# PhilipPragerUrbina/DOGERAY

Measured on AMD Instinct MI355X. Metric: Mrays/sec + ms/frame, 1M-tri .rts at 1920x1080, higher is better.
Workload: dtype f32

## Files before the change

### dogeray_amd/csrc/context.cpp

```cpp
#include <climits>
#include <exception>

#include "context.hpp"
#include "linearise.hpp"

using namespace dr;

namespace {

constexpr int ANY = INT_MIN;
struct Option { const char* name; int dr_context::*member; int lo, hi; unsigned only; bool reorders; };
const Option OPTIONS[] = {
    {"kernel", &dr_context::kernel, DR_KERNEL_TILE, DR_KERNEL_PERSISTENT, 0, false},
    {"occupancy", &dr_context::occupancy, 4, 6, 0, false},
    {"schedule", &dr_context::schedule, 0, 2, 0, false},
    {"heavy_factor", &dr_context::heavy_factor, -1, 1000, 0, true},
    {"coop_steps", &dr_context::coop_steps, 0, INT_MAX, 0, false},
    {"coop_lanes", &dr_context::coop_lanes, 1, 64, 0, false},
    {"split_parts", &dr_context::split_parts, 1, 8, 1u << 1 | 1u << 2 | 1u << 4 | 1u << 8, false},
    {"split_waves", &dr_context::split_waves, 1, 1000, 0, true},
    {"split_steps", &dr_context::split_steps, 16, 4080, 0, true},
    {"short_one_queue", &dr_context::short_one_queue, ANY, 0, 0, true},
    {"coop_rounds", &dr_context::coop_rounds, 1, 16, 0, false},
    {"reserve_cus", &dr_context::reserve_cus, 0, 64, 0, false},
    {"wave_log", &dr_context::wave_log_on, 0, 1, 0, false},
    {"coop_tiles_per_wave", &dr_context::coop_tiles_per_wave, 0, INT_MAX, 0, false},
    {"pipe_streams", &dr_context::pipe_streams, 2, dr_context::PIPE_STREAMS, 0, false},
    {"pipe_lean", &dr_context::pipe_lean, ANY, 0, 0, false},
    {"pipe_group", &dr_context::pipe_group, 1, dr_context::PIPE_GROUP_MAX, 0, false},
    {"xcd_regions", &dr_context::xcd_regions, ANY, 0, 0, true},
    {"batch_frames", &dr_context::batch_frames, 1, 256, 0, false},
    {"feedback", &dr_context::feedback, ANY, 0, 0, true},
    {"order_follows_camera", &dr_context::order_follows_camera, ANY, 0, 0, false},
    {"feedback_every", &dr_context::feedback_every, 1, INT_MAX, 0, false},
    {"wide_tree", &dr_context::wide_tree, 0, 2, 0, false},
    {"denoise_tiles", &dr_context::denoise_tiles, 0, 1, 0, false},
    {"moments", &dr_context::moments_opt, 0, 1, 0, false},
    {"denoise_variance", &dr_context::denoise_variance, 0, 1, 0, false},
    {"camera_cert", &dr_context::camera_cert, 0, 1, 0, false},
    {"cert_factor", &dr_context::cert_factor, 1, 10000, 0, false},
    {"cert_levels",  &dr_context::cert_levels, 0, 1, 0, false},
    {"camera_entry",  &dr_context::camera_entry, 0, 1, 0, false},
    {"sky_tiles",  &dr_context::sky_tiles, 0, 1, 0, false},
    {"trace_kernel",  &dr_context::trace_kernel, 0, 2, 0, false},
};

const Option* find_option(const std::string& name) {
  for (const Option& o : OPTIONS) if (name == o.name) return &o;
  return nullptr;
}

int set_option(dr_context* c, const std::string& name, int v) {
  const Option* o = find_option(name);
  if (!o) { set_error("unknown option '" + name + "'"); return DR_ERR_INVALID; }
  if (o->lo == ANY) v = v != 0;
  else if (v < o->lo || v > o->hi || (o->only && !(o->only >> v & 1u))) { set_error("value not supported for option '" + name + "'"); return DR_ERR_INVALID; }
  if (name == "split_steps") v &= ~15;
  else if (name == "wave_log") {
    if (v && !c->wave_log) {
      if (hipSetDevice(c->device) != hipSuccess || c->wave_log.alloc((size_t)WAVE_LOG_WAVES * 16) != DR_OK) { set_error("cannot allocate the wave log"); return DR_ERR_DEVICE; }
      (void)hipMemsetAsync(c->wave_log, 0, c->wave_log.n * sizeof(unsigned long long), c->stream);
    }
  }
  else if (name == "pipe_streams") {
    if (v != c->pipe_streams) {
      if (hipSetDevice(c->device) != hipSuccess || join_pipeline(c) != DR_OK || hipStreamSynchronize(c->stream) != hipSuccess) { set_error("pipe_streams: cannot drain the pipeline"); return DR_ERR_DEVICE; }
      for (int k = 0; k < dr_context::PIPE_DEPTH; k++) { c->pipe_slot[k].drained = true; c->pipe_slot[k].count = 0; }
      c->pipe_next = 0; c->pipe_groups = 0;
    }
  }
  else if (name == "camera_cert" || name == "cert_factor" || o->member == &dr_context::cert_levels || o->member == &dr_context::camera_entry ||
           o->member == &dr_context::sky_tiles) {
    if (!c->pipe_pending.empty()) DR_TRY(pipeline_flush(c));
    c->cert_valid = false;
  }
  c->*(o->member) = v;
// ... 298 lines not shown
```

### dogeray_amd/csrc/context.hpp

```cpp
#pragma once
#include <hip/hip_runtime_api.h>

#include <cmath>
#include <cstring>
#include <string>
#include <vector>

#include "kernels.hpp"
#include "params_host.hpp"
#include "scene_host.hpp"

#define HIP_TRY(expr)                                                                      \
  do {                                                                                     \
    hipError_t e_ = (expr);                                                                \
    if (e_ != hipSuccess) {                                                                \
      dr::set_error(std::string(#expr) + ": " + hipGetErrorString(e_));                    \
      return DR_ERR_DEVICE;                                                                \
    }                                                                                      \
  } while (0)

#define DR_TRY(expr)                                                                       \
  do {                                                                                     \
    const int rc_ = (expr);                                                                \
    if (rc_ != DR_OK) return rc_;                                                          \
// ... 20 lines not shown
    if (p) { HIP_TRY(hipStreamSynchronize(stream)); release(); }
    const hipError_t e = PINNED ? hipHostMalloc((void**)&p, need * sizeof(T), hipHostMallocDefault) : hipMalloc((void**)&p, need * sizeof(T));
    if (e != hipSuccess) { p = nullptr; set_error(std::string("cannot allocate ") + std::to_string(need * sizeof(T)) + " bytes: " + hipGetErrorString(e)); return DR_ERR_DEVICE; }
    n = need;
    return DR_OK;
  }
  int alloc(size_t count) { release(); return grow(count ? count : 1, nullptr); }
  int upload(const std::vector<T>& src) { DR_TRY(alloc(src.size())); return put(src.data(), src.size()); }
  int put(const T* src, size_t count) { if (count) HIP_TRY(hipMemcpy(p, src, count * sizeof(T), hipMemcpyHostToDevice)); return DR_OK; }
  int get(T* dst, size_t count) const { if (count) HIP_TRY(hipMemcpy(dst, p, count * sizeof(T), hipMemcpyDeviceToHost)); return DR_OK; }
};

struct GuideKey {
  bool valid = false;
  float st[13] = {0};
  int W = 0, H = 0;
  uint64_t gen = 0;
  bool matches(const float* settings13, int w, int h, uint64_t scene_gen) const {
    return valid && W == w && H == h && gen == scene_gen && memcmp(st, settings13, sizeof(st)) == 0;
  }
  void store(const float* settings13, int w, int h, uint64_t scene_gen) {
    memcpy(st, settings13, sizeof(st));
    W = w; H = h; gen = scene_gen; valid = true;
  }
};

struct LaunchSite {
  hipStream_t stream;
  bool hold_order;
  bool lean;
};

constexpr int TILE_COUNTERS = 1024;

}

struct dr_context {
  template <class T> using DevMem = dr::DevMem<T>;
  int device = 0;
  hipStream_t stream = nullptr;
  hipEvent_t ev0 = nullptr, ev1 = nullptr;
  hipEvent_t pev0[2] = {nullptr, nullptr}, pev1[2] = {nullptr, nullptr};
  bool pending[2] = {false, false}; uint64_t pending_frames[2] = {0, 0}, pending_samples[2] = {0, 0}; int pending_next = 0;
  DevMem<dr::DevUnit> walk; size_t walk_bytes = 0;
  DevMem<dr::DevUnit> wide; size_t wide_bytes = 0; int wide_depth = 0, wide_nodes = 0; float wide_pmax = 0; dr::WideMu wide_mu = {0, 0, 0}; int wide_own_bounds = 0;
  int wide_tree = 2;
  DevMem<dr::DevPair> pairs;
  DevMem<dr::DevPrim> prims;
  DevMem<dr::DevShade> shade;
  DevMem<dr::DevTex> tex;
  DevMem<uint32_t> texels;
  int n_prims = 0, n_tex = 0, tree_depth = 0;
  std::vector<int> slot_to_orig;
  DevMem<int32_t> slot_to_orig_dev;
  DevMem<uint8_t> aov_staging;
  DevMem<uint32_t> trace_hit;
  DevMem<unsigned> trace_cursor;
  DevMem<uint8_t> trace_staging;
  int trace_kernel = 0;
  DevMem<float> dn_planes;
  dr::GuideKey dn_key;
  DevMem<uint8_t> dn_staging;
  DevMem<float> up_planes;
  dr::GuideKey up_key;
  int up_passes = 0;
  uint64_t scene_gen = 0;
  DevMem<int32_t> accum2;
  DevMem<int32_t> hist_buf[2];
  int32_t* hist = nullptr; int hist_cur = 0;
  DevMem<float> rp_planes[2];
  dr::GuideKey rp_key; int rp_cur = 0;
  DevMem<unsigned long long> rp_counts;
  int rp_passes = 0;
  int moments_opt = 0;
  int denoise_variance = 0;
  DevMem<unsigned long long> m2_buf[2];
  unsigned long long* m2 = nullptr; int m2_cur = 0;
  DevMem<unsigned long long> err_counts;
  DevMem<float> err_staging;
  int denoise_tiles = 1;
  int camera_cert = 1;
  int cert_factor = 40;
  int cert_levels = 1;
  DevMem<uint32_t> cert_mask;
  DevMem<uint32_t> cert_level;
  bool cert_valid = false;
  bool cert_ok = false;
  bool entry_ok = false;
  float cert_key[22] = {0};
  float cert_seen[22] = {0};
  float cert_k[dr::CERT_MAX_LEVELS + 1] = {1};
  int cert_tiles = 0;
  int camera_entry = 1;
  DevMem<uint32_t> wide_leaf_rec, wide_range;
  int wide_leaves = 0;
  DevMem<uint32_t> entry_mm;
  DevMem<uint32_t> cert_word;
  int sky_tiles = 1;
  DevMem<int> launch_order, launch_region_start, sky_list;
  DevMem<unsigned> sky_counts;
  bool sky_split_last = false;
  uint64_t cert_gen = 0;
  uint64_t order_gen = 0;
  uint64_t sky_key[5] = {0, 0, 0, 0, 0}; bool sky_key_valid = false;
  DevMem<int32_t> frame;
  DevMem<int32_t> accum; int accW = 0, accH = 0;
  DevMem<uint8_t> present;
  DevMem<int32_t> packed[2];
  DevMem<unsigned long long> counters;
  DevMem<unsigned> tile_counters; int tile_cursor = 0; int num_cus = 256;
  DevMem<unsigned> pixel_cost, tile_cost; DevMem<int> tile_order, region_start;
  int order_capacity = 0;
  bool order_valid = false;
  int order_age = 0;
  int order_follows_camera = 1;
  int feedback_every = 8;
  float order_key[18] = {0};
  int order_args[5] = {0, 0, 0, 0, 0};
  int feedback = 1;
  int stripe_mod = 1, stripe_rem = 0;
  int traversal = DR_TRAVERSAL_WIDE;
  int count = 0;
  int kernel = DR_KERNEL_PERSISTENT;
  int occupancy = 6;
  int schedule = 0;
  int xcd_regions = 1;
  int heavy_factor = 1;
  int coop_steps = 2;
  int coop_tiles_per_wave = 32;
  int coop_lanes = 8;
  int split_parts = 4;
// ... 58 lines not shown
```

### dogeray_amd/csrc/context_pipeline.cpp

```cpp
#include "context.hpp"

namespace dr {

int join_pipeline(dr_context* c) {
  if (!c->pipe_pending.empty()) DR_TRY(pipeline_flush(c));
  if (!c->pipe_dirty) return DR_OK;
  for (int k = 0; k < dr_context::PIPE_DEPTH; k++) {
    const dr_context::PipeSlot& sl = c->pipe_slot[k];
    if (sl.count > 0) HIP_TRY(hipStreamWaitEvent(c->stream, sl.added[sl.count - 1], 0));
  }
  for (int k = 1; k < dr_context::PIPE_STREAMS; k++) if (c->pipe_last_set[k]) HIP_TRY(hipStreamWaitEvent(c->stream, c->pipe_last[k], 0));
  c->pipe_dirty = false;
  return DR_OK;
}

}

using namespace dr;

namespace {

int pipeline_setup(dr_context* c) {
  if (c->pipe_ready) return DR_OK;
  bool ok = c->acc_stream || hipStreamCreateWithFlags(&c->acc_stream, hipStreamNonBlocking) == hipSuccess;
// ... 41 lines not shown
    HIP_TRY(hipEventRecord(c->pipe_sync, c->stream));
    for (int q = 1; q < dr_context::PIPE_STREAMS; q++) HIP_TRY(hipStreamWaitEvent(c->pipe_stream[q], c->pipe_sync, 0));
    HIP_TRY(hipStreamWaitEvent(c->acc_stream, c->pipe_sync, 0));
    c->pipe_dirty = true;
  }
  if (!sl.drained && sl.count > 0) { HIP_TRY(hipEventSynchronize(sl.added[sl.count - 1])); sl.drained = true; }
  if (sl.count > 0) HIP_TRY(hipStreamWaitEvent(rs, sl.added[sl.count - 1], 0));
  if (sl.elems_each != elems || sl.cap_frames < n || !sl.frames) {
    const int cap = n > c->pipe_group ? n : c->pipe_group;
    sl.cap_frames = 0;
    DR_TRY(sl.frames.grow((size_t)cap * elems, c->acc_stream));
    sl.elems_each = elems; sl.cap_frames = cap;
    sl.rect[0] = -1;
  }
  const int rect[6] = {W, H, P.gx, P.gy, P.stripe_mod, P.stripe_rem};
  if (memcmp(rect, sl.rect, sizeof(rect)) != 0) {
    HIP_TRY(hipMemsetAsync(sl.frames, 0, (size_t)sl.cap_frames * elems * sizeof(int32_t), rs));
    memcpy(sl.rect, rect, sizeof(rect));
  }
  P.out = sl.frames;
  P.accumulate = 0;
  P.batch = n; P.batch_seed_stride = stride;
  P.out_frame_stride = n > 1 ? (uint32_t)elems : 0u;
  const int tiles = P.ncols * P.gy;
  bool refresh = false;
  if (c->feedback && uses_persistent(c) && tiles > 0) {
    float geom[5];
    order_geometry(P, geom);
    refresh = !c->order_valid || c->order_capacity < tiles || memcmp(c->order_key + 13, geom, sizeof(geom)) != 0 || c->order_age < 2 ||
              c->order_age % (4 * c->feedback_every) == 0;
  }
  site.hold_order = !refresh;
  if (c->pipe_barrier_set) HIP_TRY(hipStreamWaitEvent(rs, c->pipe_barrier, 0));
  const bool alone = refresh || c->tile_cursor + MAX_REGIONS > TILE_COUNTERS;
  if (alone)
    for (int q = 0; q < dr_context::PIPE_STREAMS; q++) if (q != si && c->pipe_last_set[q]) HIP_TRY(hipStreamWaitEvent(rs, c->pipe_last[q], 0));
  if (tiles > 0) {
    DR_TRY(enqueue_frame(c, site, P));
    HIP_TRY(hipGetLastError());
  }
  HIP_TRY(hipEventRecord(c->pipe_last[si], rs)); c->pipe_last_set[si] = true;
  if (alone) { HIP_TRY(hipEventRecord(c->pipe_barrier, rs)); c->pipe_barrier_set = true; }
  HIP_TRY(hipEventRecord(sl.rendered, rs));
  HIP_TRY(hipStreamWaitEvent(c->acc_stream, sl.rendered, 0));
  for (int f = 0; f < n; f++) {
    if (c->m2) launch_moments_add(c->acc_stream, c->accum, sl.frames + (size_t)f * elems, c->m2, (size_t)W * H);
    else launch_frame_add(c->acc_stream, c->accum, sl.frames + (size_t)f * elems, elems);
    const int div = c->pipe_pending[(size_t)f].div;
    sl.div[f] = 0; sl.fwaited[f] = false;
    if (div != 0) {
      const size_t bytes = (size_t)W * H * 3;
      DR_TRY(sl.rgb_dev[f].grow(bytes, c->acc_stream));
      DR_TRY(sl.rgb_host[f].grow(bytes, c->acc_stream));
      launch_present(c->acc_stream, c->accum, c->hist, sl.rgb_dev[f], W, H, div);
      HIP_TRY(hipMemcpyAsync(sl.rgb_host[f], sl.rgb_dev[f], bytes, hipMemcpyDeviceToHost, c->acc_stream));
      sl.div[f] = div;
    }
    HIP_TRY(hipGetLastError());
    HIP_TRY(hipEventRecord(sl.added[f], c->acc_stream));
  }
  sl.first = first_ticket; sl.count = n; sl.drained = false;
  c->pipe_groups = g + 1;
  c->stats.launches += tiles > 0 ? 1 : 0;
  c->stats.frames += (uint64_t)n;
  c->stats.samples += (uint64_t)(tiles > 0 ? tiles : 0) * 64ull * (uint64_t)(P.spp_f > 0 ? ceilf(P.spp_f) : 0) * (uint64_t)n;
  c->pipe_pending.erase(c->pipe_pending.begin(), c->pipe_pending.begin() + n);
  return DR_OK;
// ... 89 lines not shown
```

### dogeray_amd/csrc/context_render.cpp

```cpp
#include "context.hpp"

namespace dr {

void fill_scene(const dr_context* c, RenderParams& P) {
  P.walk = c->walk; P.walk_bytes = (uint32_t)c->walk_bytes; P.pairs = c->pairs; P.prims = c->prims; P.shade = c->shade; P.tex = c->tex; P.texels = c->texels;
  P.wide = c->wide; P.wide_bytes = (uint32_t)c->wide_bytes; P.wide_pmax = c->wide_pmax; P.wide_mu = c->wide_mu;
}

static int tiles_per_wave(const dr_context* c, const LaunchSite& site) {
  return site.lean ? 0 : c->coop_tiles_per_wave;
}

int make_params(dr_context* c, const LaunchSite& site, const float* st, int W, int H, float background, uint64_t seed, RenderParams& P, int batch_hint) {
  if (!c->walk) { set_error("no scene uploaded"); return DR_ERR_INVALID; }
  memset(&P, 0, sizeof(P));
  if (const char* why = fill_view_params(st, W, H, background, seed, c->stripe_mod, c->stripe_rem, P)) { set_error(why); return DR_ERR_INVALID; }
  if (P.backtex >= c->n_tex) { set_error("backtex refers to a texture that is not loaded"); return DR_ERR_INVALID; }
  memcpy(c->cur_settings, st, sizeof(c->cur_settings));
  fill_scene(c, P);
  P.counters = c->counters;
  P.wave_log = c->wave_log_on ? c->wave_log.p : nullptr;
  P.coop_steps = c->coop_steps; P.coop_rounds = c->coop_rounds; P.split_parts = c->split_parts;
  P.coop_lanes = c->coop_lanes;
  const int tiles = P.ncols * P.gy;
// ... 43 lines not shown
  memcpy(key, c->cur_settings, 13 * sizeof(float));
  key[13] = (float)P.W; key[14] = (float)P.H; key[15] = (float)P.stripe_mod; key[16] = (float)P.stripe_rem; key[17] = (float)P.ncols; key[18] = (float)P.gy;
  key[19] = (float)(c->scene_gen & 0xffffff); key[20] = (float)c->cert_factor; key[21] = (float)(c->cert_levels + 2 * c->camera_entry + 4 * c->camera_cert);
  if (!(c->cert_valid && memcmp(c->cert_key, key, sizeof(key)) == 0)) {
    if (site.hold_order) return;
    if (P.batch < 2 && memcmp(c->cert_seen, key, sizeof(key)) != 0) { memcpy(c->cert_seen, key, sizeof(key)); return; }
    const double a_star = 1e-4 * (double)c->cert_factor;
    CertView cv;
    c->cert_valid = false;
    c->cert_ok = c->entry_ok = false;
    c->cert_gen++;
    if (fill_cert_view(P, a_star, want_cert ? c->wide_mu.e : 1.0f, cv)) {
      if (c->cert_level.grow(cert_level_words(tiles), site.stream) != DR_OK || c->cert_word.grow((size_t)tiles, site.stream) != DR_OK ||
          (want_entry && c->entry_mm.grow(entry_mm_words(tiles), site.stream) != DR_OK)) return;
      for (float& k : c->cert_k) k = 1.0f;
      if (want_cert) {
        cert_ladder(c->cert_factor, c->cert_levels != 0, cv);
        if (c->cert_mask.grow(cert_mask_words(tiles, cv.n_levels), site.stream) != DR_OK) return;
        launch_cert_mask(site.stream, c->prims, c->n_prims, cv, c->cert_mask, c->cert_level, tiles);
        for (int g = 1; g <= CERT_MAX_LEVELS; g++) c->cert_k[g] = g <= cv.n_levels ? cert_factor_k(cv.level_a[g - 1]) : 1.0f;
      } else {
        (void)hipMemsetAsync(c->cert_level, 0, cert_level_words(tiles) * sizeof(uint32_t), site.stream);
      }
      launch_camera_entry(site.stream, c->wide, c->wide_leaf_rec, c->wide_range, c->wide_leaves, cv, want_entry ? c->entry_mm.p : nullptr, c->cert_level, c->cert_word, tiles);
      c->cert_ok = want_cert; c->entry_ok = want_entry;
    }
    memcpy(c->cert_key, key, sizeof(key));
    c->cert_tiles = tiles;
    c->cert_valid = true;
  }
  if (c->cert_ok || c->entry_ok) { P.cert_level = c->cert_word; memcpy(P.wide_cert_k, c->cert_k, sizeof(P.wide_cert_k)); }
}

bool sky_split(dr_context* c, const LaunchSite& site, const RenderParams& P, int tiles, const int*& order, const int*& region_start, unsigned* pcost) {
  if (!c->sky_tiles || !c->entry_ok || !P.cert_level || site.hold_order || site.stream != c->stream || P.out_frame_stride != 0) return false;
  if (P.max_depth <= 0 || !(P.spp_f > 0.0f)) return false;
  if (!plan_sky_split(plan_persistent(persistent_cfg(c, site), (long long)tiles * P.batch, P.coop_steps, false, P.wave_log != nullptr))) return false;
  const uint64_t key[5] = {c->cert_gen, order ? 1u : 0u, order ? c->order_gen : 0u, (uint64_t)tiles, (uint64_t)P.regions};
  const bool room = c->launch_order.n >= (size_t)tiles && c->sky_list.n >= (size_t)tiles && c->launch_region_start.p && c->sky_counts.p;
  if (!(room && c->sky_key_valid && memcmp(c->sky_key, key, sizeof(key)) == 0)) {
    c->sky_key_valid = false;
    if (c->launch_order.grow((size_t)tiles, site.stream) != DR_OK || c->sky_list.grow((size_t)tiles, site.stream) != DR_OK ||
        c->launch_region_start.grow(2 * MAX_REGIONS + 1, site.stream) != DR_OK || c->sky_counts.grow(2, site.stream) != DR_OK)
      return false;
    launch_sky_split(site.stream, order, region_start, P.region_start, P.cert_level, tiles, P.regions, c->launch_order, c->launch_region_start, c->sky_list, c->sky_counts);
    memcpy(c->sky_key, key, sizeof(key));
    c->sky_key_valid = true;
  }
  launch_sky_tiles(site.stream, P, c->sky_list, c->sky_counts, pcost);
  order = c->launch_order; region_start = c->launch_region_start;
  return true;
}

}

int enqueue_frame(dr_context* c, const LaunchSite& site, const RenderParams& P_in) {
  RenderParams P = P_in;
  const int tiles = P.ncols * P.gy;
  if (uses_persistent(c)) {
    if (c->tile_cursor + MAX_REGIONS > TILE_COUNTERS) {
      (void)hipMemsetAsync(c->tile_counters, 0, TILE_COUNTERS * sizeof(unsigned), site.stream);
      c->tile_cursor = 0;
    }
    unsigned* counter = c->tile_counters + c->tile_cursor;
    c->tile_cursor += MAX_REGIONS;
    const int* order; unsigned* pcost;
    if (site.hold_order) {
      float geom[5];
      order_geometry(P, geom);
      order = (c->order_valid && c->order_capacity >= tiles && memcmp(c->order_key + 13, geom, sizeof(geom)) == 0) ? c->tile_order.p : nullptr;
      pcost = nullptr;
    } else feedback_buffers(c, site, P, tiles, order, pcost);
    if (!c->wave_log_on) P.wave_log = nullptr;
    cert_prepare(c, site, P, tiles);
    const int* launch_order = order; const int* launch_rstart = c->region_start;
    c->sky_split_last = sky_split(c, site, P, tiles, launch_order, launch_rstart, pcost);
    const int log_waves = launch_persistent_kernel(site.stream, P, persistent_cfg(c, site), counter, launch_order, launch_rstart, pcost);
    if (log_waves < 0) { set_error("the persistent kernel has no build for this launch (launch_plan.hpp)"); return DR_ERR_DEVICE; }
    c->wave_log_waves = log_waves;
    if (pcost && !order) c->order_age = 0;
    if (pcost && (c->order_age < 2 || c->order_age % c->feedback_every == 0)) {
      const int split_limit = plan_split_limit(c->num_cus, c->occupancy, c->split_parts, c->split_waves);
      launch_tile_feedback(site.stream, c->pixel_cost, c->tile_cost, c->tile_order, c->region_start, tiles, P.regions, c->heavy_factor, c->split_steps, split_limit);
      c->order_gen++;
      c->order_args[0] = tiles; c->order_args[1] = P.regions; c->order_args[2] = c->heavy_factor; c->order_args[3] = c->split_steps; c->order_args[4] = split_limit;
      c->order_valid = true;
    }
    c->order_age++;
    return DR_OK;
  }
  c->sky_split_last = false;
  launch_tile_kernel(site.stream, P, traversal_of(c), c->count != 0, c->occupancy);
  return DR_OK;
}

}

using namespace dr;

namespace {

int launch_render(dr_context* c, const RenderParams& P) {
  int tiles = P.ncols * P.gy;
  if (tiles <= 0) return DR_OK;
  HIP_TRY(hipEventRecord(c->ev0, c->stream));
  DR_TRY(enqueue_frame(c, c->own_site(), P));
  HIP_TRY(hipGetLastError());
  HIP_TRY(hipEventRecord(c->ev1, c->stream));
  return DR_OK;
// ... 116 lines not shown
```

### dogeray_amd/csrc/device_layout.h

```cpp
#pragma once
#include <stdint.h>

namespace dr {

struct DevUnit {
  float f[4];
};
constexpr int WALK_UNITS_INTERNAL = 2;
constexpr int WALK_UNITS_LEAF = 4;
constexpr int WALK_SLOT_BITS = 26;
constexpr int WALK_KIND_SPHERE = 0, WALK_KIND_TRIANGLE = 1, WALK_KIND_NONE = 2;

inline uint32_t wide_node_first_child(const uint32_t* w) { return w[3] & 0xffffffu; }
inline uint32_t wide_node_valid(const uint32_t* w) { return (w[3] >> 24) & 15u; }
inline uint32_t wide_node_leaf_mask(const uint32_t* w) { return w[3] >> 28; }
inline uint32_t wide_node_lo(const uint32_t* w, int axis) { return w[4 + axis]; }
inline uint32_t wide_node_hi(const uint32_t* w, int axis) { return w[7 + axis]; }
inline uint32_t wide_node_scale24_bits(const uint32_t* w, int axis) { return axis == 0 ? w[10] << 16 : (axis == 1 ? w[10] & 0xffff0000u : w[11]); }
struct WideMu {
  float e;
  float l;
  float v;
};
struct CertView {
// ... 84 lines not shown
  const DevShade* shade;
  const DevTex* tex;
  const uint32_t* texels;
  int32_t* out;
  unsigned long long* counters;
  unsigned long long* wave_log;
  float from[3], llc[3], hor[3], ver[3], uu[3], vu[3];
  float lens_radius;
  float bgint;
  float scale;
  float spp_f;
  double den_w, den_h;
  uint64_t seed;
  int32_t W, H;
  int32_t gx, gy;
  int32_t ncols;
  int32_t stripe_mod, stripe_rem;
  uint32_t seed_stride;
  int32_t max_depth;
  int32_t backtex;
  int32_t accumulate;
  int32_t batch;
  uint64_t batch_seed_stride;
  int32_t coop_steps;
  int32_t coop_lanes;
  int32_t split_parts;
  int32_t coop_rounds;
  int32_t regions;
  uint32_t out_frame_stride;
  int32_t region_start[9];
  WideMu wide_mu;
  float wide_cert_k[CERT_MAX_LEVELS + 1];
  const uint32_t* cert_level;
};

constexpr int DN_MISS = -1;
constexpr int DN_OUTSIDE = -2147483647 - 1;
constexpr int DN_MAX_ITERATIONS = 10;
constexpr int DN_MAX_NORMAL_POWER_LOG2 = 16;
struct DnParams {
  int iterations;
  float sigma_luminance;
  int normal_power_log2;
  float sigma_depth;
  int demodulate;
  int material_stop;
};

constexpr int UP_BLOCK = 0, UP_GUIDED = 1;
struct UpParams {
  int mode;
  int normal_power_log2;
  float sigma_depth;
  int demodulate;
  int material_stop;
};

constexpr int RP_VALID = 0, RP_MASKED = 1, RP_OFFSCREEN = 2, RP_REJECTED = 3;
constexpr int RP_MAX_HISTORY = 65535;
struct RpParams {
  int max_history;
  float normal_cos;
  float plane_tolerance;
  uint32_t material_mask;
  int sky;
};
// ... 19 lines not shown
```

### dogeray_amd/csrc/device_sky.hpp

```cpp
#pragma once
#include "device_shade.hpp"
#include "launch_plan.hpp"

namespace dr {

__host__ __device__ __forceinline__ bool sky_word(uint32_t word) { return ((int)word >> ENTRY_SHIFT) == ENTRY_NONE; }

__device__ __forceinline__ void sky_pixel(const RenderParams& P, int x, int y, int frame, int& r, int& g, int& b) {
  V3 color = mk(0, 0, 0);
  Ctr c = {0, 0, 0, 0, 0, 0, 0, 0};
  for (int s = 0; (float)s < P.spp_f; ++s) {
    Xorwow rng;
    rng.init(sample_seed(P, x, y, s, frame));
    Path path; path.atten = splat(1.0f);
    camera_ray(P, x, y, rng, path.rayo, path.raydir);
    color = color + shade_miss<false>(P, path, c);
  }
  r = f2i(color.x * 255 * P.scale); g = f2i(color.y * 255 * P.scale); b = f2i(color.z * 255 * P.scale);
}

inline int sky_split_plain(const int* order, const int* region_start, const uint32_t* word, int tiles, int regions, int* launch_order,
                           int* launch_region_start, int* sky_list) {
  int n_geometry = 0, n_sky = 0, r = 0;
  for (int k = 0; k < 2 * MAX_REGIONS + 1; k++) launch_region_start[k] = 0;
  for (int i = 0; i < tiles; i++) {
    while (r <= regions && region_start[r] <= i) launch_region_start[r++] = n_geometry;
    const int t = order ? order[i] : i;
    if (!sky_word(word[t])) launch_order[n_geometry++] = t;
    if (sky_word(word[i])) sky_list[n_sky++] = i;
  }
  while (r <= regions) launch_region_start[r++] = n_geometry;
  return n_sky;
}

}
```

### dogeray_amd/csrc/kernels_aux.hip

```cpp
#include <hip/hip_runtime.h>

#include "device_rng.hpp"
#include "device_wide.hpp"
#include "device_cert.hpp"
#include "device_surface.hpp"
#include "device_sky.hpp"
#include "kernels.hpp"
#include "../../include/dogeray_amd.h"

namespace dr {

__global__ __launch_bounds__(256) void tile_cost_kernel(const unsigned* __restrict__ pixel_cost, unsigned* __restrict__ tile_cost, int ntiles) {
  int tile = blockIdx.x * 4 + (threadIdx.x >> 6);
  if (tile >= ntiles) return;
  unsigned v = pixel_cost[(size_t)tile * 64 + (threadIdx.x & 63)];
  for (int off = 32; off > 0; off >>= 1) { unsigned o = __shfl_xor(v, off, 64); v = o > v ? o : v; }
  if ((threadIdx.x & 63) == 0) tile_cost[tile] = v;
}
constexpr int ORDER_BUCKETS = 256;
__device__ __forceinline__ unsigned block_exclusive_scan(unsigned v, unsigned& total) {
  __shared__ unsigned wave_sum[16];
  const int lane = threadIdx.x & 63, w = threadIdx.x >> 6;
  unsigned x = v;
  for (int off = 1; off < 64; off <<= 1) { const unsigned y = __shfl_up(x, off, 64); if (lane >= off) x += y; }
// ... 153 lines not shown
      for (int k = 0; k < GROUPS; k++) {
        const int i = g0 + 64 * k + lane;
        if (g0 + 64 * k < w1) body(i, t[k], i < w1 && !sky_word(wt[k]), i < w1 && sky_word(wi[k]));
      }
    }
  };
  {
    unsigned ng = 0, ns = 0;
    for_range([&](int, int, bool geometry, bool sky) { ng += (unsigned)__popcll(__ballot(geometry)); ns += (unsigned)__popcll(__ballot(sky)); });
    if (lane == 0) { geo_cnt[w] = ng; sky_cnt[w] = ns; }
  }
  __syncthreads();
  unsigned gbase = 0, sbase = 0, gtotal = 0, stotal = 0;
  for (int k = 0; k < WAVES; k++) {
    if (k < w) { gbase += geo_cnt[k]; sbase += sky_cnt[k]; }
    gtotal += geo_cnt[k]; stotal += sky_cnt[k];
  }
  for_range([&](int i, int t, bool geometry, bool sky) {
    const unsigned long long bg = __ballot(geometry), bs = __ballot(sky);
    const unsigned p = gbase + mbcnt(bg);
    if (i < w1)
      for (int r = 0; r <= regions; r++) if (i == rs[r]) launch_region_start[r] = (int)p;
    if (geometry) launch_order[p] = t;
    if (sky) sky_list[sbase + mbcnt(bs)] = i;
    gbase += (unsigned)__popcll(bg); sbase += (unsigned)__popcll(bs);
  });
  if (tid <= regions && rs[tid] >= ntiles) launch_region_start[tid] = (int)gtotal;
  if (tid == 0) { counts[0] = stotal; counts[1] = gtotal; }
}
__global__ __launch_bounds__(256) void sky_tiles_kernel(RenderParams P, const int* __restrict__ sky_list, const unsigned* __restrict__ counts,
                                                         unsigned* __restrict__ pixel_cost) {
  const int i = blockIdx.x * 4 + (threadIdx.x >> 6), lane = threadIdx.x & 63;
  if (i >= (int)counts[0]) return;
  const int tile = sky_list[i];
  const int col = tile / P.gy, by = tile - col * P.gy;
  const int x = (P.stripe_rem + col * P.stripe_mod) * 8 + (lane >> 3), y = by * 8 + (lane & 7);
  int r = 0, g = 0, b = 0;
  for (int frame = 0; frame < P.batch; frame++) {
    int fr, fg, fb;
    sky_pixel(P, x, y, frame, fr, fg, fb);
    r += fr; g += fg; b += fb;
  }
  int32_t* px = P.out + ((size_t)x * (size_t)P.H + (size_t)y) * 3;
  if (P.accumulate == 2) { atomicAdd(px + 0, r); atomicAdd(px + 1, g); atomicAdd(px + 2, b); }
  else if (P.accumulate) { px[0] += r; px[1] += g; px[2] += b; }
  else { px[0] = r; px[1] = g; px[2] = b; }
  if (pixel_cost) pixel_cost[(size_t)tile * 64 + lane] = 0u;
}

__global__ void present_kernel(const int32_t* acc, const int32_t* hist, uint8_t* rgb, int W, int H, int div) {
  int idx = blockIdx.x * blockDim.x + threadIdx.x;
  if (idx >= W * H) return;
  int x = idx / H, y = idx - x * H;
  const int32_t* p = acc + (size_t)idx * 3;
  uint8_t* q = rgb + ((size_t)y * W + x) * 3;
  if (hist) {
    div += hist[idx];
    if (div == 0) { q[0] = 0; q[1] = 0; q[2] = 0; return; }
  }
  for (int k = 0; k < 3; k++) {
    int v = p[k] / div;
    v = v < 0 ? 0 : (v > 255 ? 255 : v);
    q[k] = (uint8_t)v;
  }
}

__global__ __launch_bounds__(256) void stripe_copy_kernel(int4* __restrict__ dst, const int4* __restrict__ src, int ncols, int run4,
                                                          long long dst_first4, long long dst_stride4, long long src_first4, long long src_stride4) {
  const int col = blockIdx.y;
  if (col >= ncols) return;
  int4* d = dst + dst_first4 + (long long)col * dst_stride4;
  const int4* sp = src + src_first4 + (long long)col * src_stride4;
  for (int i = blockIdx.x * blockDim.x + threadIdx.x; i < run4; i += gridDim.x * blockDim.x) d[i] = sp[i];
}

__global__ __launch_bounds__(256, 5) void gather_probe_kernel(RenderParams P, unsigned nrec, int iters, unsigned* out) {
  const WalkRsrc r = wide_rsrc(P);
  unsigned x = (blockIdx.x * 256u + threadIdx.x) * 2654435761u + 12345u;
  unsigned acc = 0;
  for (int i = 0; i < iters; i++) {
// ... 332 lines not shown
```

### dogeray_amd/csrc/kernels_render.hip

```cpp
#include <hip/hip_runtime.h>

#include "device_core.hpp"
#include "device_coop.hpp"
#include "kernels.hpp"
#include "../../include/dogeray_amd.h"

namespace dr {

template <bool COUNT, int MODE, int OCC>
__global__ __launch_bounds__(256, OCC) void render_kernel(RenderParams P) {
  __shared__ int lds_stack[MODE == DR_TRAVERSAL_ORDERED ? ORDERED_STACK * 256 : (MODE == DR_TRAVERSAL_WIDE ? WIDE_STACK * 256 : 1)];
  const int wave = threadIdx.x >> 6, lane = threadIdx.x & 63;
  const int tile = blockIdx.x * 4 + wave;
  Ctr c = {0, 0, 0, 0, 0, 0, 0, 0};
  if (tile < P.ncols * P.gy) {
    const int col = tile / P.gy, by = tile - col * P.gy;
    const int bx = P.stripe_rem + col * P.stripe_mod;
    const int x = bx * 8 + (lane >> 3), y = by * 8 + (lane & 7);
    if (MODE == DR_TRAVERSAL_ORDERED) {
      int* stack = lds_stack + wave * (ORDERED_STACK * 64) + lane;
      auto closest = [&](V3 o, V3 d, Ctr& cc) { return closest_hit_ordered<COUNT>(P.pairs, P.prims, o, d, cc, stack); };
      render_pixel<COUNT>(P, closest, x, y, c);
    } else if (MODE == DR_TRAVERSAL_WIDE) {
      const WalkRsrc wide = wide_rsrc(P);
      int* stack = lds_stack + wave * (WIDE_STACK * 64) + lane;
      auto closest = [&](V3 o, V3 d, Ctr& cc) { return closest_hit_wide<COUNT>(wide, P.wide_pmax, P.wide_mu.e, P.wide_mu.l, P.wide_mu.v, o, d, cc, stack); };
      render_pixel<COUNT>(P, closest, x, y, c);
    } else {
      const WalkRsrc walk = walk_rsrc(P);
      auto closest = [&](V3 o, V3 d, Ctr& cc) { return closest_hit_threaded<COUNT>(walk, o, d, cc); };
      render_pixel<COUNT>(P, closest, x, y, c);
    }
  }
  if (COUNT) {
    unsigned v[8] = {c.rays, c.V, c.L, c.S, c.T, c.samples, c.trav_slots, c.ray_slots};
    for (int k = 0; k < 8; k++) {
      unsigned long long s = v[k];
      for (int off = 32; off > 0; off >>= 1) s += __shfl_xor(s, off, 64);
      if (lane == 0 && s) atomicAdd(&P.counters[STAT_RAYS + k], s);
    }
  }
}


constexpr int PCODE_SPLIT = (int)0x80000000, PCODE_MASK = 0x7fffffff;
constexpr int SHARE_ALONE = -1, SHARE_OWNER = 64;
enum WideStashWord { WS_TOP = 0, WS_W1, WS_COLOR_X, WS_COLOR_Y, WS_COLOR_Z, WS_XY, WS_PCODE, WS_SAMPLE, WS_STEPS, WS_RSTART, WS_BOUNCE = WS_RSTART };
constexpr int WS_W1_SP_BYTE = 0, WS_W1_GRADE_BYTE = 1, WS_W1_FRAME_HALF = 1;
constexpr int XCH_OFF = (WIDE_STACK + WS_STEPS) * 64, XCH_MAX = 16, XCH_FIELDS = 8;
enum XchField { XCH_OX = 0, XCH_OY, XCH_OZ, XCH_DX, XCH_DY, XCH_DZ, XCH_WORD, XCH_ROOT };
static_assert(WS_RSTART + 1 == WIDE_STASH && XCH_MAX * XCH_FIELDS == (WIDE_STASH - WS_STEPS) * 64 && XCH_ROOT + 1 == XCH_FIELDS, "stash layout");
enum ThreadedStashWord { TS_V0X = 0, TS_C, TS_D = TS_C + 4, TS_INFO = TS_D + 4, TS_PARKED, TS_INV_X, TS_INV_Y, TS_INV_Z, TS_COLOR_X, TS_COLOR_Y, TS_COLOR_Z, TS_PX, TS_PY,
                         TS_PCODE, TS_FRAME, TS_SAMPLE, TS_STEPS, TS_RSTART, TS_WORDS };
static_assert(TS_WORDS * 64 == WAVE_LDS_DWORDS, "stash layout");

template <bool COUNT, int OCC, int TRAV_MIN, int PARK_MIN, int P_UNROLL, bool WIDE, bool COOP = true, bool PERFRAME = false>
__global__ __launch_bounds__(256, OCC) void render_persistent_kernel(RenderParams P, unsigned* __restrict__ tile_counter,
                                                                     const int* __restrict__ tile_order, const int* __restrict__ region_start,
                                                                     unsigned* __restrict__ pixel_cost) {
  const int lane = threadIdx.x & 63;
  const int wave_id = blockIdx.x * 4 + (threadIdx.x >> 6);
  constexpr int SHARE_OFF = (WIDE_STACK + WIDE_STASH) * 64;
  constexpr int REGION = WIDE ? (WIDE_STACK + WIDE_STASH + (COOP ? 3 : 0)) * 64 : WAVE_LDS_DWORDS;
  __shared__ __attribute__((aligned(16))) int wave_lds[4 * REGION];
  int* const my_lds = wave_lds + (threadIdx.x >> 6) * REGION;
  int* const my_stack = my_lds + lane;
  unsigned long long* const share_key = reinterpret_cast<unsigned long long*>(my_lds + (WIDE ? SHARE_OFF : 0));
  unsigned* const share_pend = reinterpret_cast<unsigned*>(my_lds + (WIDE ? SHARE_OFF : 0) + 128);
  if (WIDE) {
    int* const st0 = my_lds + WIDE_STACK * 64 + lane;
    for (int k = WS_W1; k < WS_STEPS; k++) st0[k * 64] = 0;
  }
  int share = SHARE_ALONE;
  WideStack ws; ws.top = 0u; ws.sp = 0; ws.sb = 0;
  const int ntiles = P.ncols * P.gy;
  const int nwork = ntiles * P.batch;
  const WalkRsrc walk = WIDE ? wide_rsrc(P) : walk_rsrc(P);
  Ctr c = {0, 0, 0, 0, 0, 0, 0, 0};
  int cur_tile = ntiles, cur_frame = 0;
  unsigned cur_cert = 0u;
  int cur_next = 64;
  int cur_limit = 64;
  bool cur_split = false;
  const bool splitting = WIDE && COOP && region_start && P.split_parts > 1 && P.batch == 1;
  int region = 0, regions_left = P.regions;
  if (P.regions > 1) region = (int)(__builtin_amdgcn_s_getreg(20 | (0 << 6) | (3 << 11)) % (unsigned)P.regions);
  (void)nwork;
  Trav tr; tr.node = LANE_REFILL; tr.best_t = 0; tr.best_slot = -1;
  Path path; path.rayo = mk(0, 0, 0); path.raydir = mk(0, 0, 0); path.atten = mk(0, 0, 0);
  V3 inv = mk(0, 0, 0), color = mk(0, 0, 0);
  WideRay wr = wide_ray_none();
  SignMask sg = sign_mask(inv);
  Xorwow rng; rng.v0 = rng.v1 = rng.v2 = rng.v3 = rng.v4 = rng.d = 0;
  int px = -1, py = 0, sample = 0, bounce = 0;
// ... 353 lines not shown
        const unsigned long long nodes2 = __ballot(tr.node >= 0 && !(tr.node & 1));
        const bool do_leaves2 = leaves2 != 0ull && ((int)__popcll(leaves2) >= park_thr || nodes2 == 0ull || draining);
        const bool do_nodes2 = !EXCLUSIVE || !do_leaves2 || draining;
        if (COUNT) { n_leafstep += do_leaves2; n_nodestep += nodes2 != 0ull && do_nodes2; }
        if (tr.node >= 0 && (at_leaf2 ? do_leaves2 : do_nodes2)) {
          if (COUNT) { if (first_active_lane()) c.trav_slots += 64; }
          const WideRec r = wide_fetch(walk, tr.node);
          if (at_leaf2) wide_leaf_compute<COUNT>(r, path.rayo, path.raydir, inv, sg, tr, ws, my_stack, c);
          else wide_node_compute<COUNT>(r, wr, sg, tr, ws, my_stack, c);
          steps++;
        }
      }
    } else if (PARK_MIN > 0) {
      const unsigned long long parked = __ballot(pk.parked);
      const unsigned long long steppers = __ballot(tr.node >= 0 && !pk.parked);
      if (parked != 0ull && (__popcll(parked) >= PARK_MIN || steppers == 0ull || cur_tile >= ntiles)) {
        if (pk.parked) parked_test<COUNT>(path.rayo, path.raydir, tr, pk, c);
      }
      for (int u = 0; u < P_UNROLL; u++) {
        if (tr.node >= 0 && !pk.parked) {
          if (COUNT) { if (first_active_lane()) c.trav_slots += 64; }
          trav_step_park<COUNT>(walk, path.rayo, inv, tr, pk, c);
          steps++;
        }
      }
    } else {
      if (tr.node >= 0) {
        if (COUNT) { if (first_active_lane()) c.trav_slots += 64; }
        trav_step<COUNT>(walk, path.rayo, path.raydir, inv, tr, c);
        steps++;
      }
    }
  }
  if (lane == 0) {
    const unsigned long long r_end = __builtin_amdgcn_s_memrealtime();
    atomicAdd(&P.counters[STAT_WAVE_CYCLES], __builtin_readcyclecounter() - t_begin);
    atomicAdd(&P.counters[STAT_WAVE_TICKS], r_end - r_begin);
    if (WAVE_LOG && P.wave_log) {
      unsigned long long* const w = P.wave_log + (size_t)wave_id * 16;
      w[0] = r_begin; w[1] = r_empty; w[2] = r_end; w[3] = n_after;
    }
  }
  if (COUNT && lane == 0) {
    atomicAdd(&P.counters[STAT_PHASE_CYCLES], t_phase);
    atomicAdd(&P.counters[STAT_ITERATIONS], n_iter);
    atomicAdd(&P.counters[STAT_PHASES], n_phase);
    atomicAdd(&P.counters[STAT_NODE_STEPS], n_nodestep);
    atomicAdd(&P.counters[STAT_LEAF_STEPS], n_leafstep);
    atomicAdd(&P.counters[STAT_SHADED], n_shaded);
    atomicAdd(&P.counters[STAT_PB_CANDS], pb_cands);
    atomicAdd(&P.counters[STAT_PB_TURNS], pb_turns);
    atomicAdd(&P.counters[STAT_PB_SPHERE], pb_sphere);
    atomicAdd(&P.counters[STAT_PB_DISK], pb_disk);
    atomicAdd(&P.counters[STAT_PB_RETIRED], pb_retired);
  }
  if (COUNT) {
    unsigned v[8] = {c.rays, c.V, c.L, c.S, c.T, c.samples, c.trav_slots, c.ray_slots};
    for (int k = 0; k < 8; k++) {
      unsigned long long s = v[k];
      for (int off = 32; off > 0; off >>= 1) s += __shfl_xor(s, off, 64);
      if (lane == 0 && s) atomicAdd(&P.counters[STAT_RAYS + k], s);
    }
  }
}

namespace {
// ... 40 lines not shown
```

### dogeray_amd/csrc/launch_plan.hpp

```cpp
#pragma once
#include "../../include/dogeray_amd.h"
#include "device_layout.h"

namespace dr {

constexpr int MAX_REGIONS = 8;
constexpr int WAVE_LOG_WAVES = 16384;

struct PersistentCfg {
  int traversal;
  int occupancy;
  int schedule;
  int num_cus;
  int coop_tiles_per_wave;
  bool count;
};

struct PersistentBuild { int count, occ, trav_min, park_min, unroll, wide, coop, perframe; };
inline bool operator==(const PersistentBuild& a, const PersistentBuild& b) {
  return a.count == b.count && a.occ == b.occ && a.trav_min == b.trav_min && a.park_min == b.park_min && a.unroll == b.unroll && a.wide == b.wide &&
         a.coop == b.coop && a.perframe == b.perframe;
}

#define DR_SCHEDULE_0 32, 20, 2, 12, 4
// ... 29 lines not shown
  return cfg.traversal == DR_TRAVERSAL_WIDE && !cfg.count && cfg.schedule == 0 && cfg.occupancy >= 6;
}

inline PersistentPlan plan_persistent(const PersistentCfg& cfg, long long work, int coop_steps, bool per_frame, bool wave_log_on) {
  const PersistentSchedule& s = PERSISTENT_SCHEDULES[cfg.schedule == 0 ? 0 : cfg.schedule == 1 ? 1 : 2];
  const bool wide = cfg.traversal == DR_TRAVERSAL_WIDE, six = persistent_can_store_per_frame(cfg);
  per_frame = per_frame && six;
  auto blocks_for = [&](int occ) {
    const int blocks = cfg.num_cus * occ;
    return (long long)blocks * 4 > work ? (int)((work + 3) / 4) : blocks;
  };
  PersistentPlan p;
  if (six && !(coop_steps > 0 && short_launch(work, cfg.coop_tiles_per_wave, (long long)cfg.num_cus * 5 * 4))) {
    p.build = {false, 6, s.trav_min, s.park_min, s.unroll, true, false, per_frame};
    p.blocks = blocks_for(6);
    p.log_waves = 0; p.clear_wave_log = true;
    return p;
  }
  const int occ = cfg.occupancy >= 5 ? 5 : 4;
  p.blocks = blocks_for(occ);
  p.clear_wave_log = wave_log_on && p.blocks * 4 > WAVE_LOG_WAVES;
  p.log_waves = wave_log_on && !p.clear_wave_log ? p.blocks * 4 : 0;
  const bool coop = per_frame || (coop_steps > 0 && short_launch(work, cfg.coop_tiles_per_wave, (long long)p.blocks * 4));
  if (!wide) p.build = {cfg.count, occ, s.trav_min, s.park_min, s.unroll, false, true, false};
  else if (cfg.count) p.build = {true, occ, s.trav_min, s.park_min, s.unroll, true, false, false};
  else if (coop) p.build = {false, occ, s.trav_min, s.coop_park, s.coop_unroll, true, true, per_frame};
  else p.build = {false, occ, s.trav_min, s.park_min, s.unroll, true, false, false};
  if (wide && !coop) p.log_waves = 0;
  return p;
}

inline bool plan_sky_split(const PersistentPlan& p) { return p.build.wide && !p.build.count && !p.build.coop && !p.build.perframe; }

inline int plan_regions(int tiles, int batch_hint, bool xcd_regions, bool short_one_queue, int tiles_per_wave, int num_cus) {
  int regions = xcd_regions ? MAX_REGIONS : 1;
  if (tiles < 64 * MAX_REGIONS) regions = 1;
  if (short_one_queue && short_launch((long long)tiles * batch_hint, tiles_per_wave, (long long)num_cus * 5 * 4)) regions = 1;
  return regions;
}

inline int plan_split_limit(int num_cus, int occupancy, int split_parts, int split_waves) {
  return split_parts > 1 ? (int)((long long)num_cus * (occupancy >= 5 ? 5 : 4) * 4 * split_waves / (100 * split_parts)) : 0;
}

enum { TRACE_KERNEL_PLAIN = 0, TRACE_KERNEL_PERSISTENT = 1 };
enum { TRACE_FORCE_NONE = 0, TRACE_FORCE_PLAIN = 1, TRACE_FORCE_PERSISTENT = 2 };
constexpr int TRACE_OCC = 6, TRACE_REFILL_MIN = 8, TRACE_PARK = 20;
constexpr int TRACE_CHUNK = 128;
constexpr long long TRACE_PERSISTENT_MIN_RAYS = 1 << 25;
struct TracePlan {
  int kernel;
  int traversal;
  int blocks;
};
inline TracePlan plan_trace(long long n, int traversal, bool has_wide, int num_cus, int force) {
  TracePlan p;
  p.traversal = (traversal == DR_TRAVERSAL_WIDE && !has_wide) ? DR_TRAVERSAL_THREADED : traversal;
  const bool can = p.traversal == DR_TRAVERSAL_WIDE;
  const bool persistent = can && (force == TRACE_FORCE_PERSISTENT || (force != TRACE_FORCE_PLAIN && n >= TRACE_PERSISTENT_MIN_RAYS));
  p.kernel = persistent ? TRACE_KERNEL_PERSISTENT : TRACE_KERNEL_PLAIN;
  if (persistent) {
    const long long full = (long long)num_cus * TRACE_OCC, need = (n + 4 * TRACE_CHUNK - 1) / (4 * TRACE_CHUNK);
    p.blocks = (int)(need < full ? need : full);
  } else p.blocks = (int)((n + 255) / 256);
  return p;
}
// ... 8 lines not shown
```

Before: 9147.

## Fold sky tile shading into persistent render kernel tail via work cursor

```diff
diff --git a/dogeray_amd/csrc/context.cpp b/dogeray_amd/csrc/context.cpp
--- a/dogeray_amd/csrc/context.cpp
+++ b/dogeray_amd/csrc/context.cpp
@@ -41,7 +41,7 @@
     {"cert_factor", &dr_context::cert_factor, 1, 10000, 0, false},
     {"cert_levels",  &dr_context::cert_levels, 0, 1, 0, false},
     {"camera_entry",  &dr_context::camera_entry, 0, 1, 0, false},
-    {"sky_tiles",  &dr_context::sky_tiles, 0, 1, 0, false},
+    {"sky_tiles",  &dr_context::sky_tiles, 0, 2, 0, false},
     {"trace_kernel",  &dr_context::trace_kernel, 0, 2, 0, false},
 };
 
diff --git a/dogeray_amd/csrc/context.hpp b/dogeray_amd/csrc/context.hpp
--- a/dogeray_amd/csrc/context.hpp
+++ b/dogeray_amd/csrc/context.hpp
@@ -76,6 +76,7 @@
 };
 
 constexpr int TILE_COUNTERS = 1024;
+constexpr int LAUNCH_COUNTERS = MAX_REGIONS + 1;
 
 }
 
@@ -140,7 +141,7 @@
   int wide_leaves = 0;
   DevMem<uint32_t> entry_mm;
   DevMem<uint32_t> cert_word;
-  int sky_tiles = 1;
+  int sky_tiles = 2;
   DevMem<int> launch_order, launch_region_start, sky_list;
   DevMem<unsigned> sky_counts;
   bool sky_split_last = false;
diff --git a/dogeray_amd/csrc/context_pipeline.cpp b/dogeray_amd/csrc/context_pipeline.cpp
--- a/dogeray_amd/csrc/context_pipeline.cpp
+++ b/dogeray_amd/csrc/context_pipeline.cpp
@@ -97,7 +97,7 @@
   }
   site.hold_order = !refresh;
   if (c->pipe_barrier_set) HIP_TRY(hipStreamWaitEvent(rs, c->pipe_barrier, 0));
-  const bool alone = refresh || c->tile_cursor + MAX_REGIONS > TILE_COUNTERS;
+  const bool alone = refresh || c->tile_cursor + LAUNCH_COUNTERS > TILE_COUNTERS;
   if (alone)
     for (int q = 0; q < dr_context::PIPE_STREAMS; q++) if (q != si && c->pipe_last_set[q]) HIP_TRY(hipStreamWaitEvent(rs, c->pipe_last[q], 0));
   if (tiles > 0) {
diff --git a/dogeray_amd/csrc/context_render.cpp b/dogeray_amd/csrc/context_render.cpp
--- a/dogeray_amd/csrc/context_render.cpp
+++ b/dogeray_amd/csrc/context_render.cpp
@@ -99,7 +99,7 @@
   if (c->cert_ok || c->entry_ok) { P.cert_level = c->cert_word; memcpy(P.wide_cert_k, c->cert_k, sizeof(P.wide_cert_k)); }
 }
 
-bool sky_split(dr_context* c, const LaunchSite& site, const RenderParams& P, int tiles, const int*& order, const int*& region_start, unsigned* pcost) {
+bool sky_split(dr_context* c, const LaunchSite& site, RenderParams& P, int tiles, const int*& order, const int*& region_start, unsigned* pcost, unsigned* cursor) {
   if (!c->sky_tiles || !c->entry_ok || !P.cert_level || site.hold_order || site.stream != c->stream || P.out_frame_stride != 0) return false;
   if (P.max_depth <= 0 || !(P.spp_f > 0.0f)) return false;
   if (!plan_sky_split(plan_persistent(persistent_cfg(c, site), (long long)tiles * P.batch, P.coop_steps, false, P.wave_log != nullptr))) return false;
@@ -114,7 +114,10 @@
     memcpy(c->sky_key, key, sizeof(key));
     c->sky_key_valid = true;
   }
-  launch_sky_tiles(site.stream, P, c->sky_list, c->sky_counts, pcost);
+  if (c->sky_tiles == 2) {
+    P.sky_list = c->sky_list; P.sky_counts = c->sky_counts; P.sky_cursor = cursor;
+    P.sky_chunk = sky_chunk_frames(P.batch, P.accumulate == 2 ? SKY_CHUNK : 0);
+  } else launch_sky_tiles(site.stream, P, c->sky_list, c->sky_counts, pcost);
   order = c->launch_order; region_start = c->launch_region_start;
   return true;
 }
@@ -125,12 +128,12 @@
   RenderParams P = P_in;
   const int tiles = P.ncols * P.gy;
   if (uses_persistent(c)) {
-    if (c->tile_cursor + MAX_REGIONS > TILE_COUNTERS) {
+    if (c->tile_cursor + LAUNCH_COUNTERS > TILE_COUNTERS) {
       (void)hipMemsetAsync(c->tile_counters, 0, TILE_COUNTERS * sizeof(unsigned), site.stream);
       c->tile_cursor = 0;
     }
     unsigned* counter = c->tile_counters + c->tile_cursor;
-    c->tile_cursor += MAX_REGIONS;
+    c->tile_cursor += LAUNCH_COUNTERS;
     const int* order; unsigned* pcost;
     if (site.hold_order) {
       float geom[5];
@@ -141,7 +144,7 @@
     if (!c->wave_log_on) P.wave_log = nullptr;
     cert_prepare(c, site, P, tiles);
     const int* launch_order = order; const int* launch_rstart = c->region_start;
-    c->sky_split_last = sky_split(c, site, P, tiles, launch_order, launch_rstart, pcost);
+    c->sky_split_last = sky_split(c, site, P, tiles, launch_order, launch_rstart, pcost, counter + MAX_REGIONS);
     const int log_waves = launch_persistent_kernel(site.stream, P, persistent_cfg(c, site), counter, launch_order, launch_rstart, pcost);
     if (log_waves < 0) { set_error("the persistent kernel has no build for this launch (launch_plan.hpp)"); return DR_ERR_DEVICE; }
     c->wave_log_waves = log_waves;
diff --git a/dogeray_amd/csrc/device_layout.h b/dogeray_amd/csrc/device_layout.h
--- a/dogeray_amd/csrc/device_layout.h
+++ b/dogeray_amd/csrc/device_layout.h
@@ -140,6 +140,10 @@
   WideMu wide_mu;
   float wide_cert_k[CERT_MAX_LEVELS + 1];
   const uint32_t* cert_level;
+  const int* sky_list;
+  const unsigned* sky_counts;
+  unsigned* sky_cursor;
+  int32_t sky_chunk;
 };
 
 constexpr int DN_MISS = -1;
diff --git a/dogeray_amd/csrc/device_sky.hpp b/dogeray_amd/csrc/device_sky.hpp
--- a/dogeray_amd/csrc/device_sky.hpp
+++ b/dogeray_amd/csrc/device_sky.hpp
@@ -19,6 +19,22 @@
   r = f2i(color.x * 255 * P.scale); g = f2i(color.y * 255 * P.scale); b = f2i(color.z * 255 * P.scale);
 }
 
+__device__ __forceinline__ void sky_tile_frames(const RenderParams& P, int tile, int lane, int first, int count, unsigned* pixel_cost) {
+  const int col = tile / P.gy, by = tile - col * P.gy;
+  const int x = (P.stripe_rem + col * P.stripe_mod) * 8 + (lane >> 3), y = by * 8 + (lane & 7);
+  int r = 0, g = 0, b = 0;
+  for (int frame = first; frame < first + count; frame++) {
+    int fr, fg, fb;
+    sky_pixel(P, x, y, frame, fr, fg, fb);
+    r += fr; g += fg; b += fb;
+  }
+  int32_t* px = P.out + ((size_t)x * (size_t)P.H + (size_t)y) * 3;
+  if (P.accumulate == 2) { atomicAdd(px + 0, r); atomicAdd(px + 1, g); atomicAdd(px + 2, b); }
+  else if (P.accumulate) { px[0] += r; px[1] += g; px[2] += b; }
+  else { px[0] = r; px[1] = g; px[2] = b; }
+  if (pixel_cost && first == 0) pixel_cost[(size_t)tile * 64 + lane] = 0u;
+}
+
 inline int sky_split_plain(const int* order, const int* region_start, const uint32_t* word, int tiles, int regions, int* launch_order,
                            int* launch_region_start, int* sky_list) {
   int n_geometry = 0, n_sky = 0, r = 0;
diff --git a/dogeray_amd/csrc/kernels_aux.hip b/dogeray_amd/csrc/kernels_aux.hip
--- a/dogeray_amd/csrc/kernels_aux.hip
+++ b/dogeray_amd/csrc/kernels_aux.hip
@@ -209,20 +209,7 @@
                                                          unsigned* __restrict__ pixel_cost) {
   const int i = blockIdx.x * 4 + (threadIdx.x >> 6), lane = threadIdx.x & 63;
   if (i >= (int)counts[0]) return;
-  const int tile = sky_list[i];
-  const int col = tile / P.gy, by = tile - col * P.gy;
-  const int x = (P.stripe_rem + col * P.stripe_mod) * 8 + (lane >> 3), y = by * 8 + (lane & 7);
-  int r = 0, g = 0, b = 0;
-  for (int frame = 0; frame < P.batch; frame++) {
-    int fr, fg, fb;
-    sky_pixel(P, x, y, frame, fr, fg, fb);
-    r += fr; g += fg; b += fb;
-  }
-  int32_t* px = P.out + ((size_t)x * (size_t)P.H + (size_t)y) * 3;
-  if (P.accumulate == 2) { atomicAdd(px + 0, r); atomicAdd(px + 1, g); atomicAdd(px + 2, b); }
-  else if (P.accumulate) { px[0] += r; px[1] += g; px[2] += b; }
-  else { px[0] = r; px[1] = g; px[2] = b; }
-  if (pixel_cost) pixel_cost[(size_t)tile * 64 + lane] = 0u;
+  sky_tile_frames(P, sky_list[i], lane, 0, P.batch, pixel_cost);
 }
 
 __global__ void present_kernel(const int32_t* acc, const int32_t* hist, uint8_t* rgb, int W, int H, int div) {
diff --git a/dogeray_amd/csrc/kernels_render.hip b/dogeray_amd/csrc/kernels_render.hip
--- a/dogeray_amd/csrc/kernels_render.hip
+++ b/dogeray_amd/csrc/kernels_render.hip
@@ -2,6 +2,7 @@
 
 #include "device_core.hpp"
 #include "device_coop.hpp"
+#include "device_sky.hpp"
 #include "kernels.hpp"
 #include "../../include/dogeray_amd.h"
 
@@ -54,12 +55,31 @@
                          TS_PCODE, TS_FRAME, TS_SAMPLE, TS_STEPS, TS_RSTART, TS_WORDS };
 static_assert(TS_WORDS * 64 == WAVE_LDS_DWORDS, "stash layout");
 
+typedef const __attribute__((address_space(4))) RenderParams* ArgBlock;
+__device__ __attribute__((noinline)) void sky_units_run(ArgBlock args, int lane, unsigned* pixel_cost) {
+#if defined(__HIP_DEVICE_COMPILE__)
+  if (args->sky_list == nullptr) return;
+  const RenderParams S = *args;
+  const unsigned n_units = sky_units(S.sky_counts[0], S.batch, S.sky_chunk);
+  __builtin_amdgcn_s_setprio(0);
+  for (;;) {
+    unsigned u = 0;
+    if (lane == 0) u = atomicAdd(S.sky_cursor, 1u);
+    u = (unsigned)__builtin_amdgcn_readfirstlane((int)u);
+    if (u >= n_units) break;
+    const SkyUnit su = sky_unit(u, S.batch, S.sky_chunk);
+    sky_tile_frames(S, S.sky_list[su.index], lane, su.first, su.count, pixel_cost);
+  }
+#endif
+}
+
 template <bool COUNT, int OCC, int TRAV_MIN, int PARK_MIN, int P_UNROLL, bool WIDE, bool COOP = true, bool PERFRAME = false>
 __global__ __launch_bounds__(256, OCC) void render_persistent_kernel(RenderParams P, unsigned* __restrict__ tile_counter,
                                                                      const int* __restrict__ tile_order, const int* __restrict__ region_start,
                                                                      unsigned* __restrict__ pixel_cost) {
   const int lane = threadIdx.x & 63;
   const int wave_id = blockIdx.x * 4 + (threadIdx.x >> 6);
+  if (WIDE && !COOP && !COUNT && !PERFRAME && P.sky_list != nullptr) __builtin_amdgcn_s_setprio(1);
   constexpr int SHARE_OFF = (WIDE_STACK + WIDE_STASH) * 64;
   constexpr int REGION = WIDE ? (WIDE_STACK + WIDE_STASH + (COOP ? 3 : 0)) * 64 : WAVE_LDS_DWORDS;
   __shared__ __attribute__((aligned(16))) int wave_lds[4 * REGION];
@@ -479,6 +499,9 @@
       }
     }
   }
+  if (WIDE && !COOP && !COUNT && !PERFRAME) {
+    sky_units_run((ArgBlock)__builtin_amdgcn_kernarg_segment_ptr(), lane, pixel_cost);
+  }
   if (lane == 0) {
     const unsigned long long r_end = __builtin_amdgcn_s_memrealtime();
     atomicAdd(&P.counters[STAT_WAVE_CYCLES], __builtin_readcyclecounter() - t_begin);
diff --git a/dogeray_amd/csrc/launch_plan.hpp b/dogeray_amd/csrc/launch_plan.hpp
--- a/dogeray_amd/csrc/launch_plan.hpp
+++ b/dogeray_amd/csrc/launch_plan.hpp
@@ -85,6 +85,20 @@
 
 inline bool plan_sky_split(const PersistentPlan& p) { return p.build.wide && !p.build.count && !p.build.coop && !p.build.perframe; }
 
+#ifndef DR_SKY_CHUNK
+#define DR_SKY_CHUNK 0
+#endif
+constexpr int SKY_CHUNK = DR_SKY_CHUNK;
+struct SkyUnit { int index, first, count; };
+constexpr int sky_chunk_frames(int batch, int chunk) { return chunk > 0 && chunk < batch ? chunk : (batch > 0 ? batch : 1); }
+constexpr int sky_chunks(int batch, int chunk) { return batch > 0 ? (batch + sky_chunk_frames(batch, chunk) - 1) / sky_chunk_frames(batch, chunk) : 0; }
+constexpr unsigned sky_units(unsigned n_sky, int batch, int chunk) { return n_sky * (unsigned)sky_chunks(batch, chunk); }
+constexpr SkyUnit sky_unit(unsigned u, int batch, int chunk) {
+  const unsigned chunks = (unsigned)sky_chunks(batch, chunk), index = u / chunks;
+  const int frames = sky_chunk_frames(batch, chunk), first = (int)(u - index * chunks) * frames;
+  return SkyUnit{(int)index, first, batch - first < frames ? batch - first : frames};
+}
+
 inline int plan_regions(int tiles, int batch_hint, bool xcd_regions, bool short_one_queue, int tiles_per_wave, int num_cus) {
   int regions = xcd_regions ? MAX_REGIONS : 1;
   if (tiles < 64 * MAX_REGIONS) regions = 1;
```

After: 9282 (median of 6 runs). 1.5% higher.
